# xubiker/deephisto

Hardware: AMD Instinct MI355X
Metric: 256x256 patches/sec WSI inference (predict_full_patched) (higher is better)
Workload: dtype bf16; 1 GPU; BASELINE configs[2]: predict_full_patched on one 50000x50000x3 closed-form synthetic WSI resident in HBM, 256x256 tiles stride 256, ResNet-18 (random init), bf16 MFMA, step = one whole slide (tile grid -> fused gather+forward -> all-gather -> ordered accumulate -> argmax); patch=256, stride=256, sampler_batch=64, micro_batch=4096, streams=1, downscale=16, n_tiles=38416, n_classes=5, parallelism=tile-range shard x1

## Files before the change

### deephisto_amd/_lib.py

```python
from __future__ import annotations

import ctypes as C
from pathlib import Path

import torch

LIB_PATH = Path(__file__).resolve().parent / "libdeephisto_hip.so"

DH_LAYOUT_NHWC, DH_LAYOUT_NCHW = 0, 1
DH_DTYPE_F32, DH_DTYPE_BF16 = 0, 1

_i32, _i64, _u32 = C.c_int32, C.c_int64, C.c_uint32
BUCKET_CB = C.CFUNCTYPE(None, C.c_int32, C.c_int64, C.c_int64, C.c_void_p)
_p = C.c_void_p

SIGNATURES = {
    "dh_abi_version": (C.c_int, []),
    "dh_last_error": (C.c_char_p, []),
    "dh_tile_grid_count": (C.c_int, [_i64, _i64, _i32, _i32, _i32, C.POINTER(_i64), C.POINTER(_i64)]),
    "dh_tile_grid": (C.c_int, [_i64, _i64, _i32, _i32, _i32, _p, _i64]),
    "dh_synth_slide": (C.c_int, [_p, _i64, _i64, _u32, _p]),
    "dh_tile_gather": (C.c_int, [_p, _i64, _i64, _p, _p, _i64, _i32, _i32, _i32, _p, _p]),
    "dh_tile_gather_aug": (C.c_int, [_p, _i64, _i64, _p, _i64, _i32, _i32, _i32, _i32, _i32, _p, _p]),
    "dh_tile_gather_raw": (C.c_int, [_p, _i64, _i64, _p, _i64, _i32, _p, _p]),
# ... 59 lines not shown
    "dh_train2_debug_act": (C.c_int, [_p, C.c_char_p, _i32, _p, _i64, _p]),
    "dh_debug_gemm1x1_bf16": (C.c_int, [_p, _p, _p, _p, _i64] + [_i32] * 8 + [_p]),
    "dh_debug_gemm1x1_fused_bf16": (C.c_int, [_p] * 7 + [_i64] + [_i32] * 8 + [_p]),
    "dh_debug_gemm1x1_bwdsums_bf16": (C.c_int, [_p] * 10 + [_i32, _p, _i64, _i32, _i32, _p]),
    "dh_debug_bn2_bf16": (C.c_int, [_p, _p, _p, _p, _i32, _p, _p, _p, _p, _i32, _p, _p, _p, _p, _i64, _i32, _p]),
    "dh_debug_stem_wgrad_bf16": (C.c_int, [_p, _p, _p, _i32, _i32, _p]),
    "dh_debug_bn2_pool_bf16": (C.c_int, [_p, _p, _p, _p, _p, _p, _p, _p, _p, _p, _p, _i32, _i32, _i32, _i32, _p]),
    "dh_debug_maxpool2_bf16": (C.c_int, [_p, _p, _p, _p, _i32, _i32, _i32, _i32, _p]),
    "dh_debug_upsample2_add_bf16": (C.c_int, [_p, _p] + [_i32] * 6 + [_p]),
    "dh_debug_avgpool_fc_dgrad2": (C.c_int, [_p, _p, _p] + [_i32] * 4 + [_p]),
    "dh_debug_wgrad_bf16": (C.c_int, [_p, _p, _p] + [_i32] * 8 + [_p]),
    "dh_debug_conv_bn_act": (C.c_int, [_p, _p, _p, _p, _p, _p] + [_i32] * 9 + [_p]),
    "dh_debug_stem_out": (C.c_int, [_p, _i64, _i32, _p, _p]),
    "dh_debug_stem_pool_bf16": (C.c_int, [_p, _p, _i64, _i64, _p, _i64, _i32, _p, _p]),
    "dh_debug_wgrad_f32": (C.c_int, [_p, _p, _p] + [_i32] * 8 + [_p]),
    "dh_debug_stem_wgrad_f32": (C.c_int, [_p, _p, _p, _i32, _i32, _p]),
    "dh_debug_dgrad_f32": (C.c_int, [_p, _p, _p, _p] + [_i32] * 7 + [_p]),
    "dh_debug_pack_f32": (C.c_int, [_p, _i32, _i32, _p, _p, _p, _p, _p]),
    "dh_debug_pack_bf16": (C.c_int, [_p, _i32, _i32, _p, _p, _p, _p, _p]),
    "dh_debug_bn_f32": (C.c_int, [_p, _p, _p, _p, _i32, _p, _p, _p, _p, _p, _p, _p, _i64, _i32, _p]),
    "dh_debug_maxpool_f32": (C.c_int, [_p, _p, _p, _p, _i32, _i32, _i32, _i32, _p]),
    "dh_debug_bn_pool_f32": (C.c_int, [_p, _p, _p, _p, _p, _p, _p, _p, _p, _i32, _i32, _i32, _i32, _p]),
    "dh_debug_stamps": (C.c_int, [_i32, _p]),
    "dh_debug_env_knobs": (C.c_int, [C.c_char_p, _i64]),
    "dh_debug_coverage_set_map": (C.c_int, [_p, _p, _p]),
    "dh_debug_resnet18_forward_tap": (C.c_int, [_p, _p, _i64, _i64, _p, _i64, _i32, C.c_char_p, _p, _i32, _p, _i64, _p, _p]),
    "dh_debug_resnet50_forward_tap": (C.c_int, [_p, _p, _i64, _i64, _p, _i64, _i32, C.c_char_p, _p, _i32, _p, _i64, _p, _p]),
    "dh_debug_resnet18_operands": (C.c_int, [_p, C.c_char_p, _p, _i64, _p, _p, _i64]),
    "dh_debug_resnet50_operands": (C.c_int, [_p, C.c_char_p, _p, _i64, _p, _p, _i64]),
}


class DeephistoHipError(RuntimeError):
    pass


_lib = None


def lib() -> C.CDLL:
    global _lib
    if _lib is None:
        if not LIB_PATH.exists():
            raise DeephistoHipError(
                f"{LIB_PATH} is missing: build it with `python -m deephisto_amd.build` "
                "(hipcc --offload-arch=gfx950). There is no CPU fallback for the HIP path.")
# ... 13 lines not shown
```

### deephisto_amd/csrc/resnet50_infer.inc

```

constexpr int R50_MAX_P = 256;
constexpr int64_t R50_MAX_TILES = ((int64_t)1 << 31) / ((int64_t)256 * (R50_MAX_P / 4) * (R50_MAX_P / 4) * 2);
static_assert(R50_MAX_TILES == DH_RESNET50_MAX_TILES, "include/deephisto_hip.h states the launch limit");

struct dh_resnet50 {
  struct Blk { int c1 = -1, c2 = -1, c3 = -1, ds = -1, stride = 1; };
  int n_classes = 0;
  std::map<std::string, std::vector<float>> params;
  std::vector<ConvLayer> convs;
  std::vector<Blk> blocks;
  float* ones = nullptr;
  float* fc_w = nullptr;
  float* fc_b = nullptr;
  bool finalized = false;
  void* ws = nullptr;
  size_t ws_bytes = 0;
  std::vector<int32_t> yx_host;
};

namespace {

void r50_topology(dh_resnet50* net) {
  net->convs.clear(); net->blocks.clear();
  auto add = [&](const std::string& n, const std::string& bn, int cin, int cout, int ks, int stride) {
// ... 61 lines not shown
  DH_LAUNCH_CHECK();
  return DH_OK;
}

int r50_forward_impl(dh_resnet50* net, const float* x, const uint8_t* slide, int64_t slide_h, int64_t slide_w, const int32_t* yx,
                     int B, int P, float* logits, hipStream_t st, Tap* tap = nullptr) {
  const int H2 = P / 4;
  auto al = [](size_t v) { return (v + 255) & ~(size_t)255; };
  const size_t px = (size_t)B * H2 * H2 * 2;
  const size_t big = al(256 * px), t1 = al(128 * px), t2 = al(64 * px);
  const size_t need = 2 * big + t1 + t2;
  if (need > net->ws_bytes) {
    if (net->ws) DH_HIP(hipFree(net->ws));
    net->ws = nullptr; net->ws_bytes = 0;
    DH_HIP(hipMalloc(&net->ws, need));
    net->ws_bytes = need;
  }
  char* base = static_cast<char*>(net->ws);
  bf16_t* X = reinterpret_cast<bf16_t*>(base);
  bf16_t* D = reinterpret_cast<bf16_t*>(base + big);
  bf16_t* T1 = reinterpret_cast<bf16_t*>(base + 2 * big);
  bf16_t* T2 = reinterpret_cast<bf16_t*>(base + 2 * big + t1);
  int rc;
  if ((rc = launch_stem_pool(net->convs[0], x, slide, slide_h, slide_w, yx, B, P, X, st))) return rc;
  for (const char* nm : {"conv1", "maxpool"})
    if ((rc = tap_after<__bf16>(tap, nm, X, 64, H2, H2, 32, st))) return rc;
  int H = H2;
  for (const dh_resnet50::Blk& b : net->blocks) {
    const ConvLayer &c1 = net->convs[b.c1], &c2 = net->convs[b.c2], &c3 = net->convs[b.c3];
    const int Ho = (H - 1) / b.stride + 1;
    if ((rc = r50_gemm(c1, X, nullptr, T1, B, H, H, true, st))) return rc;
    if ((rc = tap_after<__bf16>(tap, c1.name, T1, c1.cout, H, H, 32, st))) return rc;
    rc = b.stride == 1 ? launch_conv3x3<__bf16, 1>(c2, T1, nullptr, T2, B, H, H, true, st, Ho, Ho, nullptr, nullptr, true)
                       : launch_conv3x3<__bf16, 2>(c2, T1, nullptr, T2, B, H, H, true, st, Ho, Ho, nullptr, nullptr, true);
    if (rc) return rc;
    if ((rc = tap_after<__bf16>(tap, c2.name, T2, c2.cout, Ho, Ho, 32, st))) return rc;
    const bf16_t* idt = X;
    if (b.ds >= 0) {
      if ((rc = r50_gemm(net->convs[b.ds], X, nullptr, D, B, H, H, false, st))) return rc;
      if ((rc = tap_after<__bf16>(tap, net->convs[b.ds].name, D, c3.cout, Ho, Ho, 32, st))) return rc;
      idt = D;
    }
    if ((rc = r50_gemm(c3, T2, idt, X, B, Ho, Ho, true, st))) return rc;
    if ((rc = tap_after<__bf16>(tap, c3.name, X, c3.cout, Ho, Ho, 32, st))) return rc;
    H = Ho;
  }
  hipLaunchKernelGGL(r50_head_kernel, dim3(B), dim3(256), 0, st, X, H * H, net->fc_w, net->fc_b, net->n_classes, logits);
// ... 160 lines not shown
```

### deephisto_amd/csrc/resnet_kernels.hip

```cpp
#include <math.h>
#include <stdlib.h>
#include <string.h>

#include <algorithm>
#include <array>
#include <map>
#include <mutex>
#include <set>
#include <string>
#include <vector>

#include "dh_common.h"
#include "conv3_tables_host.h"

typedef float f32x16 __attribute__((ext_vector_type(16)));
typedef __bf16 bf16x8 __attribute__((ext_vector_type(8)));

namespace {

constexpr int CHUNK_BYTES = 64;
constexpr int PIX_PITCH = 80;
constexpr int FRAG_BYTES = 1024;
constexpr int SLAB_TAP = 4 * FRAG_BYTES;

// ... 997 lines not shown
int run_conv(const ConvLayer& L, const void* in, const void* res, void* out, int B, int Hi, int Wi,
             bool relu, hipStream_t st, int* Ho_out, int* Wo_out, bool blocked = false, bool out16 = false) {
  const int pad = L.ks / 2;
  const int Ho = (Hi + 2 * pad - L.ks) / L.stride + 1, Wo = (Wi + 2 * pad - L.ks) / L.stride + 1;
  *Ho_out = Ho; *Wo_out = Wo;
  DH_REQUIRE((int64_t)B * Hi * Wi * L.cin * (int64_t)sizeof(T) < ((int64_t)1 << 32),
             "conv %s: input larger than 4 GiB, reduce the batch", L.name.c_str());
  if (L.ks == 3 && L.stride == 1) return launch_conv3x3<T, 1>(L, in, res, out, B, Hi, Wi, relu, st, Ho, Wo, nullptr, nullptr, blocked, 0, 0, false, out16);
  DH_REQUIRE(!out16, "conv %s: only the stride-1 3x3 kernel writes 16-channel planes", L.name.c_str());
  if (L.ks == 3 && L.stride == 2) return launch_conv3x3<T, 2>(L, in, res, out, B, Hi, Wi, relu, st, Ho, Wo, nullptr, nullptr, blocked);
  DH_REQUIRE(!blocked, "conv %s: only the 3x3 kernels read the channel-blocked layout", L.name.c_str());
  ConvParams p;
  p.in = in; p.w = L.w_dev; p.scale = L.scale_dev; p.shift = L.shift_dev; p.res = res; p.out = out;
  p.B = B; p.Hi = Hi; p.Wi = Wi; p.Cin = L.cin; p.Cout = L.cout; p.Ho = Ho; p.Wo = Wo;
  if (p.Ho > 8 || p.Wo > 8) { p.TH = 16; p.TW = 16; p.IMGS = 1; }
  else { p.TH = 8; p.TW = 8; p.IMGS = 4; }
  p.tiles_y = (p.Ho + p.TH - 1) / p.TH; p.tiles_x = (p.Wo + p.TW - 1) / p.TW;
  p.relu = relu ? 1 : 0;
  if (L.ks == 1 && L.stride == 2) return launch_conv<T, 1, 2, false>(p, st);
  dh::set_error("conv %s: unsupported shape", L.name.c_str());
  return DH_EINVAL;
}

int launch_stem_pool(const ConvLayer& stem, const float* x, const uint8_t* slide, int64_t slide_h, int64_t slide_w,
                     const int32_t* yx, int B, int P, void* out, hipStream_t st) {
  const int H1 = (P + 6 - 7) / 2 + 1, H2 = (H1 + 2 - 3) / 2 + 1;
  StemPoolParams sp;
  DH_REQUIRE(!slide || slide_w < (1 << 24), "stem: slide rows of %lld pixels are not supported (< 2^24)", (long long)slide_w);
  sp.x_nchw = x; sp.slide = slide; sp.yx = yx; sp.row_bytes = slide_w * 3; sp.slide_bytes = slide_h * slide_w * 3;
  sp.w = stem.w_dev; sp.scale = stem.scale_dev; sp.shift = stem.shift_dev; sp.out = out;
  sp.B = B; sp.P = P; sp.Hc = H1; sp.Wc = H1; sp.Hp = H2; sp.Wp = H2;
  sp.tiles_y = (H2 + SP_PR - 1) / SP_PR; sp.tiles_x = (H2 + SP_PC - 1) / SP_PC;
  sp.nstrips = B * sp.tiles_x;
  const int grid = std::min(768, sp.nstrips);
  sp.iters = ((sp.nstrips + grid - 1) / grid) * sp.tiles_y;
  int arc;
  if ((arc = ensure_dyn_lds(reinterpret_cast<const void*>(&stem_pool_kernel<true, false>), SP_LDS)) ||
      (arc = ensure_dyn_lds(reinterpret_cast<const void*>(&stem_pool_kernel<true, true>), SP_LDS)) ||
      (arc = ensure_dyn_lds(reinterpret_cast<const void*>(&stem_pool_kernel<false, false>), SP_LDS))) return arc;
  sp.stamps = nullptr;
  if (g_stamps_on && slide) {
    if (!g_stamps_dev) {
      DH_HIP(hipMalloc((void**)&g_stamps_dev, 64 * sizeof(unsigned long long)));
      DH_HIP(hipMemset(g_stamps_dev, 0, 64 * sizeof(unsigned long long)));
    }
    sp.stamps = g_stamps_dev + 8 * 7;
  }
  if (slide && sp.stamps) hipLaunchKernelGGL((stem_pool_kernel<true, true>), dim3(grid), dim3(SP_T), SP_LDS, st, sp);
  else if (slide) hipLaunchKernelGGL((stem_pool_kernel<true, false>), dim3(grid), dim3(SP_T), SP_LDS, st, sp);
  else hipLaunchKernelGGL((stem_pool_kernel<false, false>), dim3(grid), dim3(SP_T), SP_LDS, st, sp);
  DH_LAUNCH_CHECK();
  return DH_OK;
}

struct Tap {
  std::string name;
  const int32_t* sel = nullptr;
  int k = 0;
  float* out = nullptr;
  int64_t out_elems = 0;
  bool hit = false;
};

template <typename T>
__global__ void tap_gather_kernel(const T* __restrict__ in, const int32_t* __restrict__ sel, int C, int cp, int64_t hw, int64_t total,
                                  float* __restrict__ out) {
  for (int64_t i = (int64_t)blockIdx.x * blockDim.x + threadIdx.x; i < total; i += (int64_t)gridDim.x * blockDim.x) {
    const int64_t px = i % hw;
    const int c = (int)((i / hw) % C);
    const int64_t b = sel[i / hw / C];
    out[i] = (float)in[((b * (C / cp) + c / cp) * hw + px) * cp + c % cp];
  }
}

// ... 28 lines not shown
  const int esz = (int)sizeof(T);
  const int H1 = (P + 6 - 7) / 2 + 1;
  const int H2 = (H1 + 2 - 3) / 2 + 1;
  const size_t stem_bytes = (size_t)B * H1 * H1 * 64 * esz;
  const size_t act_bytes = (size_t)B * H2 * H2 * 64 * esz;
  DH_REQUIRE(act_bytes < ((size_t)1 << 32),
             "resnet18 forward: %d tiles of %d x %d in %s make an activation larger than 4 GiB: use fewer tiles per launch", B, P, P,
             sizeof(T) == 2 ? "bf16" : "float32");
  auto al = [](size_t v) { return (v + 255) & ~(size_t)255; };
  const size_t need = al(stem_bytes) + 3 * al(act_bytes);
  if (need > net->ws_bytes) {
    if (net->ws) DH_HIP(hipFree(net->ws));
    net->ws = nullptr; net->ws_bytes = 0;
    DH_HIP(hipMalloc(&net->ws, need));
    net->ws_bytes = need;
  }
  char* base = static_cast<char*>(net->ws);
  void* S = base;
  void* bufA = base + al(stem_bytes);
  void* bufB = base + al(stem_bytes) + al(act_bytes);
  void* bufC = base + al(stem_bytes) + 2 * al(act_bytes);

  if constexpr (sizeof(T) == 2) {
    if (int rc = launch_stem_pool(net->convs[0], x, slide, slide_h, slide_w, yx, B, P, bufA, st)) return rc;
    for (const char* nm : {"conv1", "maxpool"})
      if (int rc = tap_after<T>(tap, nm, bufA, 64, H2, H2, 32, st)) return rc;
  } else {
  {
    StemParams sp;
    sp.x_nchw = x; sp.slide = slide; sp.yx = yx; sp.row_bytes = slide_w * 3;
    sp.w = net->convs[0].w_dev; sp.scale = net->convs[0].scale_dev; sp.shift = net->convs[0].shift_dev;
    sp.out = S; sp.B = B; sp.P = P; sp.Ho = H1; sp.Wo = H1; sp.relu = 1;
    sp.tiles_y = (H1 + STEM_TH - 1) / STEM_TH; sp.tiles_x = (H1 + STEM_TW - 1) / STEM_TW;
    const size_t wb = esz == 2 ? (size_t)7 * 2 * 2 * FRAG_BYTES : (size_t)7 * 11 * 2 * 256;
    const size_t lds = wb + (size_t)STEM_ROWS * STEM_ROWE * esz;
    const int grid = B * sp.tiles_y * sp.tiles_x;
    if (slide) {
      if (int arc = ensure_dyn_lds(reinterpret_cast<const void*>(&stem_kernel<T, true>), 96 * 1024)) return arc;
      hipLaunchKernelGGL((stem_kernel<T, true>), dim3(grid), dim3(256), lds, st, sp);
    } else {
      if (int arc = ensure_dyn_lds(reinterpret_cast<const void*>(&stem_kernel<T, false>), 96 * 1024)) return arc;
      hipLaunchKernelGGL((stem_kernel<T, false>), dim3(grid), dim3(256), lds, st, sp);
    }
    DH_LAUNCH_CHECK();
    if (int rc = tap_after<T>(tap, "conv1", S, 64, H1, H1, 64, st)) return rc;
  }
  {
// ... 241 lines not shown
    hipLaunchKernelGGL((to_f32_kernel<__bf16>), dim3(1024), dim3(256), 0, st, static_cast<const __bf16*>(net->ws), out_dev, elems);
  DH_LAUNCH_CHECK();
  return DH_OK;
}

namespace {
__global__ void blocked_to_nhwc_f32_kernel(const __bf16* in, float* out, int64_t n, int hw) {
  const int64_t total = n * hw * 64;
  for (int64_t i = blockIdx.x * (int64_t)blockDim.x + threadIdx.x; i < total; i += (int64_t)gridDim.x * blockDim.x) {
    const int c = (int)(i % 64);
    const int64_t px = (i / 64) % hw, b = i / 64 / hw;
    out[i] = (float)in[((b * 2 + c / 32) * hw + px) * 32 + c % 32];
  }
}
}

extern "C" int dh_debug_stem_pool_bf16(dh_resnet18* net, const uint8_t* slide_dev, int64_t slide_h, int64_t slide_w,
                                       const int32_t* yx_dev, int64_t n, int32_t P, float* out_dev, void* stream) {
  DH_REQUIRE(net && net->finalized && net->dtype == DH_DTYPE_BF16, "debug stem pool: needs a finalized bf16 network");
  DH_REQUIRE(slide_dev && yx_dev && out_dev && n > 0 && n <= (1 << 20) && P >= 32 && P <= 1024, "debug stem pool: bad arguments");
  hipStream_t st = dh::as_stream(stream);
  const int H1 = (P + 6 - 7) / 2 + 1, H2 = (H1 + 2 - 3) / 2 + 1;
  void* tmp = nullptr;
  DH_HIP(hipMalloc(&tmp, (size_t)n * H2 * H2 * 64 * 2));
  int rc = launch_stem_pool(net->convs[0], nullptr, slide_dev, slide_h, slide_w, yx_dev, (int)n, P, tmp, st);
  if (!rc) {
    hipLaunchKernelGGL(blocked_to_nhwc_f32_kernel, dim3(1024), dim3(256), 0, st, static_cast<const __bf16*>(tmp), out_dev, n, H2 * H2);
    if (hipGetLastError() != hipSuccess) rc = DH_EHIP;
    (void)hipStreamSynchronize(st);
  }
  (void)hipFree(tmp);
  return rc;
}

namespace {
template <typename Net>
bool tap_name_known(const Net* net, const char* name) {
  if (!strcmp(name, "maxpool")) return true;
  for (const auto& c : net->convs)
    if (c.name == name) return true;
  return false;
}

int read_operands(const ConvLayer& c, int esz, bool fused_stem, float* w_host, int64_t w_elems, float* scale_host, float* shift_host,
                  int64_t c_elems) {
  DH_REQUIRE(w_host && scale_host && shift_host, "operands: null argument");
  DH_REQUIRE(w_elems == (int64_t)c.cout * c.cin * c.ks * c.ks && c_elems == c.cout, "operands %s: buffers of %lld / %lld elements, "
             "expected %lld / %d", c.name.c_str(), (long long)w_elems, (long long)c_elems, (long long)c.cout * c.cin * c.ks * c.ks, c.cout);
// ... 57 lines not shown
    float t = 0.f;
    DH_HIP(hipEventElapsedTime(&t, g_prof.ev[i], g_prof.ev[i + 1]));
    ms += t;
  }
  if (total_ms) *total_ms = ms;
  if (total_flops) *total_flops = g_prof.flops;
  if (n_samples) *n_samples = (int64_t)(g_prof.used / 2);
  for (hipEvent_t e : g_prof.ev) (void)hipEventDestroy(e);
  g_prof.ev.clear(); g_prof.used = 0;
  return DH_OK;
}

extern "C" int dh_debug_stamps(int32_t enable, unsigned long long* out64_host) {
  g_stamps_on = enable != 0;
  if (out64_host) {
    if (!g_stamps_dev) { memset(out64_host, 0, 64 * sizeof(unsigned long long)); return DH_OK; }
    DH_HIP(hipDeviceSynchronize());
    DH_HIP(hipMemcpy(out64_host, g_stamps_dev, 64 * sizeof(unsigned long long), hipMemcpyDeviceToHost));
    DH_HIP(hipMemset(g_stamps_dev, 0, 64 * sizeof(unsigned long long)));
  }
  return DH_OK;
}

#include "gemm1x1_f32.inc"
#include "train.inc"
#include "train2_kernels.inc"
#include "wgrad_ring.inc"
#include "bn_fold.inc"
#include "gemm1x1.inc"
#include "train2.inc"
#include "gemm1x1_infer.inc"
#include "resnet50_infer.inc"
```

### deephisto_amd/csrc/stem_pool.inc

```
#ifndef SP_ABL
#define SP_ABL 0
#endif
constexpr int SP_W = 4;
constexpr int SP_T = SP_W * 64;
constexpr int SP_CR = 2 * SP_W, SP_CC = 32;
constexpr int SP_PR = SP_W, SP_PC = 15;
constexpr int SP_WR = 2 * SP_CR + 5;
constexpr int SP_WE = 224;
#ifndef SP_PF
#define SP_PF 3
#endif
constexpr int SP_KS = 11;
constexpr int SP_WBYTES = SP_KS * 2 * FRAG_BYTES;
constexpr int SP_WINB = ((SP_WR * SP_WE * 2 + 255) / 256) * 256;
constexpr int SP_XCH = 4096;
constexpr int SP_LDS = SP_WBYTES + SP_WINB + (SP_W + 1) * SP_XCH + 512;
constexpr int SP_DW = 52;
constexpr int SP_NLOAD = (SP_WR * SP_DW + SP_T - 1) / SP_T;
static_assert(3 * ((SP_LDS + 511) / 512 * 512) <= 160 * 1024, "three workgroups per CU");

inline void sp_kslot(int ks, int hh, int j, int* kh, int* s) {
  *kh = -1; *s = 0;
  if (ks < 9) {
    const int pz = ks / 3, u = ks % 3;
    if (u == 0) { *kh = 2 * pz; *s = 8 * hh + j; }
    else if (u == 1) { *kh = 2 * pz + hh; *s = hh ? j : 16 + j; }
    else { *kh = 2 * pz + 1; *s = 8 + 8 * hh + j; }
  } else if (ks == 9) { *kh = 6; *s = 8 * hh + j; }
  else if (hh == 0) { *kh = 6; *s = 16 + j; }
}

struct StemPoolParams {
  const float* x_nchw; const uint8_t* slide; const int32_t* yx; int64_t row_bytes, slide_bytes;
  const void* w; const float* scale; const float* shift; void* out;
  int B, P, Hc, Wc, Hp, Wp, tiles_y, tiles_x, nstrips, iters;
  unsigned long long* stamps;
};

typedef unsigned short sp_u16x2 __attribute__((ext_vector_type(2)));

template <bool SRC_U8, bool STAMP>
__global__ __launch_bounds__(SP_T, 3) void stem_pool_kernel(const StemPoolParams p) {
  extern __shared__ __attribute__((aligned(16))) char smem[];
  char* w_lds = smem;
  char* win_lds = smem + SP_WBYTES;
  char* xch_lds = win_lds + SP_WINB;
  float* ss_lds = reinterpret_cast<float*>(xch_lds + (SP_W + 1) * SP_XCH);
  const int tid = threadIdx.x, lane = tid & 63, tx = lane & 31, h = lane >> 5;
  const int wave = __builtin_amdgcn_readfirstlane(tid >> 6);
  for (int i = wave; i < SP_WBYTES / 1024; i += SP_W)
    lds_dma<16>(static_cast<const char*>(p.w) + i * 1024 + lane * 16, __builtin_amdgcn_readfirstlane(lds_addr_of(w_lds + i * 1024)));
  if (tid < 128) ss_lds[tid] = tid < 64 ? p.scale[tid] : p.shift[tid - 64];
  for (int i = tid * 16; i < SP_WINB; i += SP_T * 16) *reinterpret_cast<uint4*>(win_lds + i) = make_uint4(0, 0, 0, 0);

  struct Tile { int valid, b, py0, px0, ty0, tx0, first; };
  int cur_sid = (int)blockIdx.x, cur_ty = 0, cur_b = cur_sid / p.tiles_x, cur_px0 = (cur_sid % p.tiles_x) * SP_PC, cur_it = 0;
  auto next_tile = [&]() __attribute__((always_inline)) {
    Tile t;
    t.valid = cur_sid < p.nstrips && cur_it < p.iters;
    t.b = cur_b; t.py0 = cur_ty * SP_PR; t.px0 = cur_px0; t.first = cur_ty == 0;
    t.ty0 = 0; t.tx0 = 0;
    if constexpr (SRC_U8) {
      if (t.valid) { t.ty0 = p.yx[2 * t.b]; t.tx0 = p.yx[2 * t.b + 1]; }
    }
    ++cur_it;
    if (++cur_ty == p.tiles_y) {
      cur_ty = 0; cur_sid += (int)gridDim.x;
      cur_b = cur_sid / p.tiles_x; cur_px0 = (cur_sid % p.tiles_x) * SP_PC;
    }
    return t;
  };

  constexpr int SP_TAIL = SP_WR * SP_DW - (SP_NLOAD - 1) * SP_T;
  uint32_t wr[SP_NLOAD], wr2[SP_NLOAD];
  uint32_t woff[SP_NLOAD];
  int wrd[SP_NLOAD];
  uint32_t colm[SP_NLOAD];
#pragma unroll
  for (int k = 0; k < SP_NLOAD; ++k) {
    wr[k] = 0; wr2[k] = 0; colm[k] = 0;
    const int idx = tid + k * SP_T;
    const bool own = idx < SP_WR * SP_DW;
    const int r = own ? idx / SP_DW : 0, d = own ? idx % SP_DW : 0;
    woff[k] = (uint32_t)(r * (int)p.row_bytes + 4 * d);
    wrd[k] = r << 8 | d;
  }
  struct __attribute__((packed, aligned(1))) U32 { uint32_t v; };
  auto load_window = [&](const Tile& t, uint32_t (&wr)[SP_NLOAD]) __attribute__((always_inline)) {
    if constexpr (SRC_U8) {
      const int iy0 = 4 * t.py0 - 3, ix0 = 4 * t.px0 - 5;
      const int64_t worg = (int64_t)(t.ty0 + iy0) * p.row_bytes + (int64_t)(t.tx0 + ix0) * 3 - 1;
      const int64_t wend = worg + (int64_t)(SP_WR - 1) * p.row_bytes + 4 * SP_DW;
      if constexpr (SP_ABL & 2) return;
      if (worg >= 0 && wend <= p.slide_bytes) {
        const uint8_t* base = p.slide + worg;
#pragma unroll
        for (int k = 0; k < SP_NLOAD; ++k) wr[k] = reinterpret_cast<const U32*>(base + ((SP_ABL & 64) ? (woff[k] & 1023u) : woff[k]))->v;
      } else {
#pragma unroll
        for (int k = 0; k < SP_NLOAD; ++k) {
          const int64_t a = worg + woff[k];
          uint32_t v = 0;
          for (int i = 0; i < 4; ++i)
            if (a + i >= 0 && a + i < p.slide_bytes) v |= (uint32_t)p.slide[a + i] << (8 * i);
          wr[k] = v;
        }
      }
    }
  };
  auto store_window = [&](const Tile& t, uint32_t (&wr)[SP_NLOAD]) __attribute__((always_inline)) {
    uint16_t* win = reinterpret_cast<uint16_t*>(win_lds);
    const int iy0 = 4 * t.py0 - 3, ix0 = 4 * t.px0 - 5;
    if constexpr (SRC_U8) {
      if constexpr (SP_ABL & 4) {
#pragma unroll
        for (int k = 0; k < SP_NLOAD; ++k) if (wr[k] == 0x12345678u) win[k] = 1;
        return;
      }
      if (t.first) {
        const int q_lo = max(0, -ix0) * 3, q_hi = min(207, (p.P - ix0) * 3);
#pragma unroll
        for (int k = 0; k < SP_NLOAD; ++k) {
          const int q0 = 4 * (wrd[k] & 255) - 1;
          const int lo = min(max(q_lo - q0, 0), 4), hi = min(max(q_hi - q0, 0), 4);
          colm[k] = (lo < 4 ? 0xFFFFFFFFu << (8 * lo) : 0u) & (hi > 0 ? 0xFFFFFFFFu >> (32 - 8 * hi) : 0u);
        }
      }
      if (!(ix0 >= 0 && ix0 + 69 <= p.P)) {
#pragma unroll
        for (int k = 0; k < SP_NLOAD; ++k) wr[k] &= colm[k];
      }
      if (!(iy0 >= 0 && iy0 + SP_WR <= p.P)) {
        const int r_lo = max(0, -iy0), r_hi = min(SP_WR, p.P - iy0);
#pragma unroll
        for (int k = 0; k < SP_NLOAD; ++k) {
          const int r = wrd[k] >> 8;
          if (r < r_lo || r >= r_hi) wr[k] = 0u;
        }
      }
#pragma unroll
      for (int k = 0; k < SP_NLOAD; ++k) {
        if (k < SP_NLOAD - 1 || tid < SP_TAIL) {
          const float r255 = 1.0f / 255.0f;
          const uint32_t w = wr[k];
          typedef __bf16 bf16x4_t __attribute__((ext_vector_type(4)));
          const bf16x4_t w4 = {(__bf16)((float)(w & 0xFFu) * r255), (__bf16)((float)((w >> 8) & 0xFFu) * r255),
                               (__bf16)((float)((w >> 16) & 0xFFu) * r255), (__bf16)((float)(w >> 24) * r255)};
          *reinterpret_cast<bf16x4_t*>(win + (wrd[k] >> 8) * SP_WE + 4 * (wrd[k] & 255)) = w4;
        }
      }
    } else {
      for (int idx = tid; idx < SP_WR * 207; idx += SP_T) {
        const int r = idx / 207, q = idx % 207;
        const int iy = iy0 + r, ix = ix0 + q / 3, c = q % 3;
        float v = 0.f;
        if (iy >= 0 && iy < p.P && ix >= 0 && ix < p.P) v = p.x_nchw[(((int64_t)t.b * 3 + c) * p.P + iy) * p.P + ix];
        win[r * SP_WE + 1 + q] = (uint16_t)f32_to_bf16(v);
      }
    }
  };

  Tile cur = next_tile();
  Tile nxt = next_tile();
  Tile nn = next_tile();
#ifdef SP_STAGGER
  {
    const int ph = (int)(blockIdx.x / 256u) % 3;
    for (int i = 0; i < ph * SP_STAGGER; ++i) __builtin_amdgcn_s_sleep(32);
  }
#endif
  asm volatile("s_waitcnt vmcnt(0)" ::: "memory");
  __syncthreads();
  if (cur.valid) { load_window(cur, wr); store_window(cur, wr); }
  if (nxt.valid) load_window(nxt, wr);
  __syncthreads();

  unsigned long long tacc[6] = {0, 0, 0, 0, 0, 0};
  unsigned long long tprev = STAMP ? __builtin_readcyclecounter() : 0ull;
  auto stamp = [&](int slot) __attribute__((always_inline)) {
    if constexpr (STAMP) {
      __builtin_amdgcn_sched_barrier(0);
      const unsigned long long now = __builtin_readcyclecounter();
      __builtin_amdgcn_sched_barrier(0);
      tacc[slot] += now - tprev;
      tprev = now;
    }
  };
  typedef short sp_i16x2 __attribute__((ext_vector_type(2)));
  auto max16 = [](uint32_t a, uint32_t b) __attribute__((always_inline)) {
    return __builtin_bit_cast(uint32_t, __builtin_elementwise_max(__builtin_bit_cast(sp_i16x2, a), __builtin_bit_cast(sp_i16x2, b)));
  };
  auto hmax3 = [&](uint32_t v0) __attribute__((always_inline)) {
    const uint32_t v1 = (uint32_t)__builtin_amdgcn_update_dpp(0, (int)v0, 0x130, 0xF, 0xF, true);
    const uint32_t v2 = (uint32_t)__builtin_amdgcn_update_dpp(0, (int)v1, 0x130, 0xF, 0xF, true);
    return max16(max16(v0, v1), v2);
  };
  const int xlane = lane * 64, xsw = (lane >> 2) & 3;
  const bool even = !(tx & 1);
  const char* a_base = w_lds + lane * 16;
  const int b_base = ((4 * wave) * SP_WE + 6 * tx) * 2;
  int b_off[3];
  b_off[0] = 16 * h;
  b_off[1] = h ? SP_WE * 2 : 32;
  b_off[2] = h ? 16 : 32;
  struct SpStep { int row, shift, sel, ka, kb; };
  constexpr SpStep SCHED[14] = {
      {0, 0, 0, 0, -1}, {0, 0, 1, 1, -1}, {1, 16, 0, 2, -1},
      {2, 0, 0, 3, 0},  {2, 0, 1, 4, 1},  {3, 16, 0, 5, 2},
      {4, 0, 0, 6, 3},  {4, 0, 1, 7, 4},  {5, 16, 0, 8, 5},
      {6, 0, 0, 9, 6},  {6, 0, 1, 10, 7}, {7, 16, 0, -1, 8},
      {8, 0, 0, -1, 9}, {8, 0, 2, -1, 10}};
  auto read_a = [&](int ks, int mt) __attribute__((always_inline)) {
    return (SP_ABL & 32) ? make_uint4(lane, tid, lane, lane) : *reinterpret_cast<const uint4*>(a_base + (ks * 2 + mt) * FRAG_BYTES);
  };
  auto read_b = [&](int f) __attribute__((always_inline)) {
    const uint32_t* src = reinterpret_cast<const uint32_t*>(win_lds + b_base + b_off[SCHED[f].sel] + SCHED[f].row * SP_WE * 2 + SCHED[f].shift);
    return (SP_ABL & 32) ? make_uint4(tid, tid, lane, tid) : make_uint4(src[0], src[1], src[2], src[3]);
  };
// ... 13 lines not shown
      };
#pragma unroll
      for (int f = 0; f < SP_PF; ++f) fetch(f);
#pragma unroll
      for (int f = 0; f < 14; ++f) {
        if (f + SP_PF < 14) fetch(f + SP_PF);
#pragma unroll
        for (int nt = 0; nt < 2; ++nt) {
          const int ks = nt == 0 ? SCHED[f].ka : SCHED[f].kb;
          if (ks < 0) continue;
#pragma unroll
          for (int mt = 0; mt < 2; ++mt) {
            if constexpr (SP_ABL & 1) {
              if (ks == 0) acc[mt][nt] = zero16;
              asm volatile("" :: "v"(wa[ks][mt].x), "v"(wa[ks][mt].y), "v"(wa[ks][mt].z), "v"(wa[ks][mt].w), "v"(bq[f % (SP_PF + 1)].x), "v"(bq[f % (SP_PF + 1)].y), "v"(bq[f % (SP_PF + 1)].z), "v"(bq[f % (SP_PF + 1)].w));
            } else {
              acc[mt][nt] = __builtin_amdgcn_mfma_f32_32x32x16_bf16(__builtin_bit_cast(bf16x8, wa[ks][mt]), __builtin_bit_cast(bf16x8, bq[f % (SP_PF + 1)]),
                                                                    ks == 0 ? zero16 : acc[mt][nt], 0, 0, 0);
            }
          }
        }
      }
      stamp(1);
      const int r0 = 2 * cur.py0, c0 = 2 * cur.px0 - 1;
      const bool interior = r0 + SP_CR <= p.Hc && c0 >= 0 && c0 + SP_CC <= p.Wc;
      char* slot = xch_lds + (wave < SP_W - 1 ? wave : SP_W - 1 + (it & 1)) * SP_XCH + xlane;
      auto bn_pack = [&](auto inside) __attribute__((always_inline)) {
        constexpr bool INSIDE = decltype(inside)::value;
        uint32_t okm[2] = {~0u, ~0u};
        if constexpr (!INSIDE) {
          const bool col_ok = (c0 + tx) >= 0 && (c0 + tx) < p.Wc;
          okm[0] = col_ok && (r0 + 2 * wave) < p.Hc ? ~0u : 0u;
          okm[1] = col_ok && (r0 + 2 * wave + 1) < p.Hc ? ~0u : 0u;
        }
        typedef float f32x2_t __attribute__((ext_vector_type(2)));
        typedef __bf16 bf16x2_t __attribute__((ext_vector_type(2)));
#pragma unroll
        for (int mt = 0; mt < 2; ++mt)
#pragma unroll
          for (int pr = 0; pr < 2; ++pr) {
            uint32_t rb[2][2];
#pragma unroll
            for (int gg = 0; gg < 2; ++gg) {
              const int g = 2 * pr + gg;
              const float4 sc = *reinterpret_cast<const float4*>(ss_lds + (mt * 4 + g) * 8 + 4 * h);
              const float4 sh = *reinterpret_cast<const float4*>(ss_lds + 64 + (mt * 4 + g) * 8 + 4 * h);
              uint32_t row[2][2];
// ... 6 lines not shown
                if constexpr (!INSIDE) { row[nt][0] &= okm[nt]; row[nt][1] &= okm[nt]; }
              }
              rb[gg][0] = row[1][0]; rb[gg][1] = row[1][1];
              vm[mt][g][0] = max16(row[0][0], row[1][0]);
              vm[mt][g][1] = max16(row[0][1], row[1][1]);
            }
            *reinterpret_cast<uint4*>(slot + (((mt * 2 + pr) ^ xsw) << 4)) = make_uint4(rb[0][0], rb[0][1], rb[1][0], rb[1][1]);
          }
      };
      if (interior) bn_pack(std::true_type{});
      else bn_pack(std::false_type{});
      stamp(2);
    }
    asm volatile("s_waitcnt lgkmcnt(0)" ::: "memory");
    __builtin_amdgcn_s_barrier();
    asm volatile("" ::: "memory");
    stamp(5);
    if (nxt.valid) store_window(nxt, wnow);
    stamp(4);
    if (cur.valid) {
      const char* prev = xch_lds + (wave > 0 ? wave - 1 : SP_W - 1 + ((it + 1) & 1)) * SP_XCH + xlane;
      const bool have_prev = wave > 0 || !cur.first;
      const int py = cur.py0 + wave, px = cur.px0 + (tx >> 1);
      const bool st_ok = even && (tx >> 1) < SP_PC && py < p.Hp && px < p.Wp;
      const int plane = p.Hp * p.Wp * 32;
      __bf16* out = static_cast<__bf16*>(p.out) + (int64_t)cur.b * 2 * plane + (py * p.Wp + px) * 32;
      uint4 pvq[4];
#pragma unroll
      for (int q = 0; q < 4; ++q) pvq[q] = make_uint4(0u, 0u, 0u, 0u);
      if (have_prev) {
#pragma unroll
        for (int q = 0; q < 4; ++q) pvq[q] = *reinterpret_cast<const uint4*>(prev + ((q ^ xsw) << 4));
      }
#pragma unroll
      for (int mt = 0; mt < 2; ++mt)
#pragma unroll
        for (int pr = 0; pr < 2; ++pr) {
          const uint4 pv = pvq[mt * 2 + pr];
          uint32_t v[4] = {max16(vm[mt][2 * pr][0], pv.x), max16(vm[mt][2 * pr][1], pv.y),
                           max16(vm[mt][2 * pr + 1][0], pv.z), max16(vm[mt][2 * pr + 1][1], pv.w)};
          if constexpr (!(SP_ABL & 8)) {
#pragma unroll
            for (int i = 0; i < 4; ++i) v[i] = max16(hmax3(v[i]), 0u);
          }
          uint32_t a0 = v[0], a1 = v[1], b0 = v[2], b1 = v[3];
          { const auto r = __builtin_amdgcn_permlane32_swap(a0, b0, false, false); a0 = r[0]; b0 = r[1]; }
          { const auto r = __builtin_amdgcn_permlane32_swap(a1, b1, false, false); a1 = r[0]; b1 = r[1]; }
          if constexpr (SP_ABL & 16) asm volatile("" :: "v"(a0), "v"(a1), "v"(b0), "v"(b1));
          else if (st_ok) *reinterpret_cast<uint4*>(out + mt * plane + (2 * pr + h) * 8) = make_uint4(a0, a1, b0, b1);
        }
      stamp(3);
    }
    asm volatile("s_waitcnt lgkmcnt(0)" ::: "memory");
    __builtin_amdgcn_s_barrier();
    asm volatile("" ::: "memory");
    stamp(5);
    cur = nxt;
    nxt = nn;
    nn = n3;
  };
  for (int it = 0; it < p.iters; it += 2) {
    step(it, wr, wr2);
    step(it + 1, wr2, wr);
  }
  if constexpr (STAMP) {
    if (tid == 0 && p.stamps) {
      for (int i = 0; i < 6; ++i) atomicAdd(p.stamps + i, tacc[i]);
      atomicAdd(p.stamps + 6, 1ull);
    }
  }
}
```

### include/deephisto_hip_debug.h

```cpp
#ifndef DEEPHISTO_HIP_DEBUG_H
#define DEEPHISTO_HIP_DEBUG_H

#include "deephisto_hip.h"

#ifdef __cplusplus
extern "C" {
#endif

int dh_train2_debug_act(dh_train2* net, const char* conv_name, int32_t what, float* out_dev, int64_t n_elem, void* stream);

int dh_debug_pack_bf16(const float* w_dev, int32_t cout, int32_t cin, uint16_t* wf_tile, uint16_t* wd_tile, uint16_t* wf_elem,
                       uint16_t* wd_elem, void* stream);
int dh_debug_gemm1x1_bf16(const uint16_t* a_dev, const uint16_t* w_dev, const uint16_t* res_dev, uint16_t* out_dev, int64_t M,
                          int32_t N, int32_t K, int32_t stride, int32_t Ho, int32_t Wo, int32_t Hi, int32_t Wi, int32_t repeat,
                          void* stream);
int dh_debug_gemm1x1_fused_bf16(const uint16_t* a_dev, const uint16_t* w_dev, const uint16_t* res_dev, const uint16_t* mask_dev,
                                uint16_t* out_dev, float* mean_dev, float* invstd_dev, int64_t M, int32_t N, int32_t K, int32_t stride,
                                int32_t Ho, int32_t Wo, int32_t Hi, int32_t Wi, int32_t repeat, void* stream);
int dh_debug_gemm1x1_bwdsums_bf16(const uint16_t* a_dev, const uint16_t* w_dev, const uint16_t* res_dev, const uint16_t* mask_dev,
                                  uint16_t* out_dev, const uint16_t* z_dev, const float* mean_dev, const float* invstd_dev,
                                  const float* scale_dev, const float* shift_dev, int32_t relu_mode, float* sums_dev, int64_t M, int32_t N,
                                  int32_t K, void* stream);
int dh_debug_bn2_bf16(const uint16_t* z_dev, const uint16_t* res_dev, const float* gamma_dev, const float* beta_dev, int32_t relu,
                      uint16_t* y_dev, float* mean_dev, float* invstd_dev, const uint16_t* dy_dev, int32_t relu_mode, uint16_t* dz_dev,
// ... 13 lines not shown

int dh_debug_conv_bn_act(const void* in_dev, const float* w_host, const float* scale_host,
                         const float* shift_host, const void* res_dev, void* out_dev, int32_t B,
                         int32_t H, int32_t W, int32_t cin, int32_t cout, int32_t ks, int32_t stride,
                         int32_t relu, int32_t dtype, void* stream);
int dh_debug_stem_out(dh_resnet18* net, int64_t n, int32_t patch, float* out_dev, void* stream);
int dh_debug_stem_pool_bf16(dh_resnet18* net, const uint8_t* slide_dev, int64_t slide_h, int64_t slide_w, const int32_t* yx_dev,
                            int64_t n, int32_t patch, float* out_dev, void* stream);
int dh_debug_wgrad_f32(const float* dz_dev, const float* x_dev, float* dw_dev, int32_t B, int32_t Hi, int32_t Wi,
                       int32_t cin, int32_t cout, int32_t ks, int32_t stride, int32_t mode, void* stream);
int dh_debug_stem_wgrad_f32(const float* dz_dev, const float* x_nchw_dev, float* dw_dev, int32_t B, int32_t P, void* stream);
int dh_debug_dgrad_f32(const float* dz_dev, const float* w_dev, const float* res_dev, float* dx_dev, int32_t B, int32_t Hi,
                       int32_t Wi, int32_t cin, int32_t cout, int32_t ks, int32_t stride, void* stream);
int dh_debug_pack_f32(const float* w_dev, int32_t cout, int32_t cin, float* wf_tile, float* wd_tile, float* wf_elem, float* wd_elem,
                      void* stream);
int dh_debug_bn_f32(const float* z_dev, const float* gamma_dev, const float* beta_dev, const float* res_dev, int32_t relu,
                    float* y_dev, const float* dy_dev, float* dz_dev, float* g_dev, float* dgamma_dev, float* dbeta_dev,
                    float* stats_out_dev, int64_t rows, int32_t C, void* stream);
int dh_debug_maxpool_f32(const float* x_dev, float* y_dev, const float* dy_dev, float* dx_dev, int32_t B, int32_t Hi, int32_t Wi,
                         int32_t C, void* stream);
int dh_debug_bn_pool_f32(const float* z_dev, const float* gamma_dev, const float* beta_dev, float* pooled_dev, uint8_t* idx_dev,
                         const float* dpool_dev, float* dz_dev, float* dgamma_dev, float* dbeta_dev, int32_t B, int32_t Hi, int32_t Wi,
                         int32_t C, void* stream);
int dh_debug_stamps(int32_t enable, unsigned long long* out64_host);
int dh_debug_env_knobs(char* buf_host, int64_t cap);

int dh_debug_resnet18_forward_tap(dh_resnet18* net, const uint8_t* slide, int64_t h, int64_t w, const int32_t* yx_dev, int64_t n, int32_t P,
                                  const char* conv_name, const int32_t* sel_dev, int32_t k, float* out_dev, int64_t out_elems,
                                  float* logits_dev, void* stream);
int dh_debug_resnet50_forward_tap(dh_resnet50* net, const uint8_t* slide, int64_t h, int64_t w, const int32_t* yx_dev, int64_t n, int32_t P,
                                  const char* conv_name, const int32_t* sel_dev, int32_t k, float* out_dev, int64_t out_elems,
                                  float* logits_dev, void* stream);
int dh_debug_resnet18_operands(dh_resnet18* net, const char* conv_name, float* w_host, int64_t w_elems, float* scale_host,
                               float* shift_host, int64_t c_elems);
int dh_debug_resnet50_operands(dh_resnet50* net, const char* conv_name, float* w_host, int64_t w_elems, float* scale_host,
                               float* shift_host, int64_t c_elems);

int dh_debug_coverage_set_map(dh_coverage* cov, const int32_t* map_host, void* stream);

#ifdef __cplusplus
}
#endif
#endif
```

Baseline: 220,500 patches/s.

## Use 16-column stem strips with a seam fixup pass instead of overlapping 15-column strips

The fused stem conv+BN+ReLU+maxpool kernel previously tiled pooled output into strips of 15 columns, which recomputes halo columns so each strip can pool alone. The strip width is now chosen at runtime and is 16 when that gives fewer strips, as it does for 256 patches (4 strips instead of 5 per row). Each strip then pools only its own columns. The left neighbour's contribution to the column at each strip boundary is saved in a seam scratch buffer, and a small follow-up kernel max-merges it into the output. This removes redundant stem compute and window loads, but adds a second kernel launch, extra seam scratch traffic and more index logic.

```diff
diff --git a/deephisto_amd/_lib.py b/deephisto_amd/_lib.py
--- a/deephisto_amd/_lib.py
+++ b/deephisto_amd/_lib.py
@@ -105,6 +105,7 @@
     "dh_debug_maxpool_f32": (C.c_int, [_p, _p, _p, _p, _i32, _i32, _i32, _i32, _p]),
     "dh_debug_bn_pool_f32": (C.c_int, [_p, _p, _p, _p, _p, _p, _p, _p, _p, _i32, _i32, _i32, _i32, _p]),
     "dh_debug_stamps": (C.c_int, [_i32, _p]),
+    "dh_debug_stem_strip_width": (C.c_int, [_i32]),
     "dh_debug_env_knobs": (C.c_int, [C.c_char_p, _i64]),
     "dh_debug_coverage_set_map": (C.c_int, [_p, _p, _p]),
     "dh_debug_resnet18_forward_tap": (C.c_int, [_p, _p, _i64, _i64, _p, _i64, _i32, C.c_char_p, _p, _i32, _p, _i64, _p, _p]),
diff --git a/deephisto_amd/csrc/resnet50_infer.inc b/deephisto_amd/csrc/resnet50_infer.inc
--- a/deephisto_amd/csrc/resnet50_infer.inc
+++ b/deephisto_amd/csrc/resnet50_infer.inc
@@ -107,7 +107,8 @@
   bf16_t* T1 = reinterpret_cast<bf16_t*>(base + 2 * big);
   bf16_t* T2 = reinterpret_cast<bf16_t*>(base + 2 * big + t1);
   int rc;
-  if ((rc = launch_stem_pool(net->convs[0], x, slide, slide_h, slide_w, yx, B, P, X, st))) return rc;
+  DH_REQUIRE(stem_seam_bytes(B, P) <= t1, "resnet50 forward: seam scratch larger than the bottleneck buffer");
+  if ((rc = launch_stem_pool(net->convs[0], x, slide, slide_h, slide_w, yx, B, P, X, T1, st))) return rc;
   for (const char* nm : {"conv1", "maxpool"})
     if ((rc = tap_after<__bf16>(tap, nm, X, 64, H2, H2, 32, st))) return rc;
   int H = H2;
diff --git a/deephisto_amd/csrc/resnet_kernels.hip b/deephisto_amd/csrc/resnet_kernels.hip
--- a/deephisto_amd/csrc/resnet_kernels.hip
+++ b/deephisto_amd/csrc/resnet_kernels.hip
@@ -1043,22 +1043,48 @@
   return DH_EINVAL;
 }
 
+int g_stem_pc_force = 0;
+
+int stem_pool_pc(int P) {
+  const int H1 = (P + 6 - 7) / 2 + 1, H2 = (H1 + 2 - 3) / 2 + 1;
+  if (g_stem_pc_force) return g_stem_pc_force;
+  return (H2 + 15) / 16 < (H2 + 14) / 15 ? 16 : 15;
+}
+
+size_t stem_seam_bytes(int B, int P) {
+  const int H1 = (P + 6 - 7) / 2 + 1, H2 = (H1 + 2 - 3) / 2 + 1;
+  return stem_pool_pc(P) == 16 ? (size_t)B * ((H2 + 15) / 16 - 1) * H2 * 64 * 2 : 0;
+}
+
+template <int PC>
+int launch_stem_pool_pc(const StemPoolParams& sp, int grid, hipStream_t st) {
+  int arc;
+  if ((arc = ensure_dyn_lds(reinterpret_cast<const void*>(&stem_pool_kernel<true, false, PC>), SP_LDS)) ||
+      (arc = ensure_dyn_lds(reinterpret_cast<const void*>(&stem_pool_kernel<true, true, PC>), SP_LDS)) ||
+      (arc = ensure_dyn_lds(reinterpret_cast<const void*>(&stem_pool_kernel<false, false, PC>), SP_LDS))) return arc;
+  if (sp.slide && sp.stamps) hipLaunchKernelGGL((stem_pool_kernel<true, true, PC>), dim3(grid), dim3(SP_T), SP_LDS, st, sp);
+  else if (sp.slide) hipLaunchKernelGGL((stem_pool_kernel<true, false, PC>), dim3(grid), dim3(SP_T), SP_LDS, st, sp);
+  else hipLaunchKernelGGL((stem_pool_kernel<false, false, PC>), dim3(grid), dim3(SP_T), SP_LDS, st, sp);
+  DH_LAUNCH_CHECK();
+  return DH_OK;
+}
+
 int launch_stem_pool(const ConvLayer& stem, const float* x, const uint8_t* slide, int64_t slide_h, int64_t slide_w,
-                     const int32_t* yx, int B, int P, void* out, hipStream_t st) {
+                     const int32_t* yx, int B, int P, void* out, void* seam, hipStream_t st) {
   const int H1 = (P + 6 - 7) / 2 + 1, H2 = (H1 + 2 - 3) / 2 + 1;
+  const int pc = stem_pool_pc(P);
   StemPoolParams sp;
   DH_REQUIRE(!slide || slide_w < (1 << 24), "stem: slide rows of %lld pixels are not supported (< 2^24)", (long long)slide_w);
   sp.x_nchw = x; sp.slide = slide; sp.yx = yx; sp.row_bytes = slide_w * 3; sp.slide_bytes = slide_h * slide_w * 3;
   sp.w = stem.w_dev; sp.scale = stem.scale_dev; sp.shift = stem.shift_dev; sp.out = out;
   sp.B = B; sp.P = P; sp.Hc = H1; sp.Wc = H1; sp.Hp = H2; sp.Wp = H2;
-  sp.tiles_y = (H2 + SP_PR - 1) / SP_PR; sp.tiles_x = (H2 + SP_PC - 1) / SP_PC;
+  sp.tiles_y = (H2 + SP_PR - 1) / SP_PR; sp.tiles_x = (H2 + pc - 1) / pc;
+  sp.seam = seam;
+  const int nseam = pc == 16 ? sp.tiles_x - 1 : 0;
+  DH_REQUIRE(!nseam || seam, "stem: %d strips of 16 pooled columns need a seam scratch", sp.tiles_x);
   sp.nstrips = B * sp.tiles_x;
   const int grid = std::min(768, sp.nstrips);
   sp.iters = ((sp.nstrips + grid - 1) / grid) * sp.tiles_y;
-  int arc;
-  if ((arc = ensure_dyn_lds(reinterpret_cast<const void*>(&stem_pool_kernel<true, false>), SP_LDS)) ||
-      (arc = ensure_dyn_lds(reinterpret_cast<const void*>(&stem_pool_kernel<true, true>), SP_LDS)) ||
-      (arc = ensure_dyn_lds(reinterpret_cast<const void*>(&stem_pool_kernel<false, false>), SP_LDS))) return arc;
   sp.stamps = nullptr;
   if (g_stamps_on && slide) {
     if (!g_stamps_dev) {
@@ -1067,10 +1093,13 @@
     }
     sp.stamps = g_stamps_dev + 8 * 7;
   }
-  if (slide && sp.stamps) hipLaunchKernelGGL((stem_pool_kernel<true, true>), dim3(grid), dim3(SP_T), SP_LDS, st, sp);
-  else if (slide) hipLaunchKernelGGL((stem_pool_kernel<true, false>), dim3(grid), dim3(SP_T), SP_LDS, st, sp);
-  else hipLaunchKernelGGL((stem_pool_kernel<false, false>), dim3(grid), dim3(SP_T), SP_LDS, st, sp);
-  DH_LAUNCH_CHECK();
+  if (int rc = pc == 16 ? launch_stem_pool_pc<16>(sp, grid, st) : launch_stem_pool_pc<15>(sp, grid, st)) return rc;
+  if (nseam) {
+    const int64_t total = (int64_t)B * nseam * H2 * 8;
+    hipLaunchKernelGGL(stem_seam_kernel, dim3((unsigned)((total + 255) / 256)), dim3(256), 0, st, static_cast<const void*>(seam),
+                       static_cast<__bf16*>(out), total, nseam, H2, H2);
+    DH_LAUNCH_CHECK();
+  }
   return DH_OK;
 }
 
@@ -1145,7 +1174,8 @@
   void* bufC = base + al(stem_bytes) + 2 * al(act_bytes);
 
   if constexpr (sizeof(T) == 2) {
-    if (int rc = launch_stem_pool(net->convs[0], x, slide, slide_h, slide_w, yx, B, P, bufA, st)) return rc;
+    DH_REQUIRE(stem_seam_bytes(B, P) <= al(stem_bytes), "resnet18 forward: seam scratch larger than the stem slot");
+    if (int rc = launch_stem_pool(net->convs[0], x, slide, slide_h, slide_w, yx, B, P, bufA, S, st)) return rc;
     for (const char* nm : {"conv1", "maxpool"})
       if (int rc = tap_after<T>(tap, nm, bufA, 64, H2, H2, 32, st)) return rc;
   } else {
@@ -1433,8 +1463,10 @@
   hipStream_t st = dh::as_stream(stream);
   const int H1 = (P + 6 - 7) / 2 + 1, H2 = (H1 + 2 - 3) / 2 + 1;
   void* tmp = nullptr;
-  DH_HIP(hipMalloc(&tmp, (size_t)n * H2 * H2 * 64 * 2));
-  int rc = launch_stem_pool(net->convs[0], nullptr, slide_dev, slide_h, slide_w, yx_dev, (int)n, P, tmp, st);
+  auto al = [](size_t v) { return (v + 255) & ~(size_t)255; };
+  const size_t out_bytes = al((size_t)n * H2 * H2 * 64 * 2);
+  DH_HIP(hipMalloc(&tmp, out_bytes + stem_seam_bytes((int)n, P) + 256));
+  int rc = launch_stem_pool(net->convs[0], nullptr, slide_dev, slide_h, slide_w, yx_dev, (int)n, P, tmp, static_cast<char*>(tmp) + out_bytes, st);
   if (!rc) {
     hipLaunchKernelGGL(blocked_to_nhwc_f32_kernel, dim3(1024), dim3(256), 0, st, static_cast<const __bf16*>(tmp), out_dev, n, H2 * H2);
     if (hipGetLastError() != hipSuccess) rc = DH_EHIP;
@@ -1538,6 +1570,12 @@
   return DH_OK;
 }
 
+extern "C" int dh_debug_stem_strip_width(int32_t pc) {
+  DH_REQUIRE(pc == 0 || pc == 15 || pc == 16, "debug stem strip width: %d is not 0, 15 or 16", pc);
+  g_stem_pc_force = pc;
+  return DH_OK;
+}
+
 #include "gemm1x1_f32.inc"
 #include "train.inc"
 #include "train2_kernels.inc"
diff --git a/deephisto_amd/csrc/stem_pool.inc b/deephisto_amd/csrc/stem_pool.inc
--- a/deephisto_amd/csrc/stem_pool.inc
+++ b/deephisto_amd/csrc/stem_pool.inc
@@ -4,7 +4,7 @@
 constexpr int SP_W = 4;
 constexpr int SP_T = SP_W * 64;
 constexpr int SP_CR = 2 * SP_W, SP_CC = 32;
-constexpr int SP_PR = SP_W, SP_PC = 15;
+constexpr int SP_PR = SP_W;
 constexpr int SP_WR = 2 * SP_CR + 5;
 constexpr int SP_WE = 224;
 #ifndef SP_PF
@@ -33,14 +33,17 @@
 struct StemPoolParams {
   const float* x_nchw; const uint8_t* slide; const int32_t* yx; int64_t row_bytes, slide_bytes;
   const void* w; const float* scale; const float* shift; void* out;
+  void* seam;
   int B, P, Hc, Wc, Hp, Wp, tiles_y, tiles_x, nstrips, iters;
   unsigned long long* stamps;
 };
 
 typedef unsigned short sp_u16x2 __attribute__((ext_vector_type(2)));
 
-template <bool SRC_U8, bool STAMP>
+template <bool SRC_U8, bool STAMP, int PC>
 __global__ __launch_bounds__(SP_T, 3) void stem_pool_kernel(const StemPoolParams p) {
+  static_assert(PC == 15 || PC == 16, "strips of 15 or 16 pooled columns");
+  constexpr int CX = 16 - PC;
   extern __shared__ __attribute__((aligned(16))) char smem[];
   char* w_lds = smem;
   char* win_lds = smem + SP_WBYTES;
@@ -54,7 +57,7 @@
   for (int i = tid * 16; i < SP_WINB; i += SP_T * 16) *reinterpret_cast<uint4*>(win_lds + i) = make_uint4(0, 0, 0, 0);
 
   struct Tile { int valid, b, py0, px0, ty0, tx0, first; };
-  int cur_sid = (int)blockIdx.x, cur_ty = 0, cur_b = cur_sid / p.tiles_x, cur_px0 = (cur_sid % p.tiles_x) * SP_PC, cur_it = 0;
+  int cur_sid = (int)blockIdx.x, cur_ty = 0, cur_b = cur_sid / p.tiles_x, cur_px0 = (cur_sid % p.tiles_x) * PC, cur_it = 0;
   auto next_tile = [&]() __attribute__((always_inline)) {
     Tile t;
     t.valid = cur_sid < p.nstrips && cur_it < p.iters;
@@ -66,7 +69,7 @@
     ++cur_it;
     if (++cur_ty == p.tiles_y) {
       cur_ty = 0; cur_sid += (int)gridDim.x;
-      cur_b = cur_sid / p.tiles_x; cur_px0 = (cur_sid % p.tiles_x) * SP_PC;
+      cur_b = cur_sid / p.tiles_x; cur_px0 = (cur_sid % p.tiles_x) * PC;
     }
     return t;
   };
@@ -74,7 +77,7 @@
   constexpr int SP_TAIL = SP_WR * SP_DW - (SP_NLOAD - 1) * SP_T;
   uint32_t wr[SP_NLOAD], wr2[SP_NLOAD];
   uint32_t woff[SP_NLOAD];
-  int wrd[SP_NLOAD];
+  uint32_t wdst[SP_NLOAD];
   uint32_t colm[SP_NLOAD];
 #pragma unroll
   for (int k = 0; k < SP_NLOAD; ++k) {
@@ -83,12 +86,17 @@
     const bool own = idx < SP_WR * SP_DW;
     const int r = own ? idx / SP_DW : 0, d = own ? idx % SP_DW : 0;
     woff[k] = (uint32_t)(r * (int)p.row_bytes + 4 * d);
-    wrd[k] = r << 8 | d;
+    wdst[k] = (uint32_t)((r * SP_WE + 4 * d) * 2);
   }
+  auto piece_rd = [&](int k, int* r, int* d) __attribute__((always_inline)) {
+    uint32_t w = wdst[k];
+    asm volatile("" : "+v"(w));
+    *r = (int)(w / (uint32_t)(SP_WE * 2)); *d = (int)(w % (uint32_t)(SP_WE * 2)) >> 3;
+  };
   struct __attribute__((packed, aligned(1))) U32 { uint32_t v; };
   auto load_window = [&](const Tile& t, uint32_t (&wr)[SP_NLOAD]) __attribute__((always_inline)) {
     if constexpr (SRC_U8) {
-      const int iy0 = 4 * t.py0 - 3, ix0 = 4 * t.px0 - 5;
+      const int iy0 = 4 * t.py0 - 3, ix0 = 4 * t.px0 - 2 * CX - 3;
       const int64_t worg = (int64_t)(t.ty0 + iy0) * p.row_bytes + (int64_t)(t.tx0 + ix0) * 3 - 1;
       const int64_t wend = worg + (int64_t)(SP_WR - 1) * p.row_bytes + 4 * SP_DW;
       if constexpr (SP_ABL & 2) return;
@@ -110,7 +118,7 @@
   };
   auto store_window = [&](const Tile& t, uint32_t (&wr)[SP_NLOAD]) __attribute__((always_inline)) {
     uint16_t* win = reinterpret_cast<uint16_t*>(win_lds);
-    const int iy0 = 4 * t.py0 - 3, ix0 = 4 * t.px0 - 5;
+    const int iy0 = 4 * t.py0 - 3, ix0 = 4 * t.px0 - 2 * CX - 3;
     if constexpr (SRC_U8) {
       if constexpr (SP_ABL & 4) {
 #pragma unroll
@@ -121,7 +129,9 @@
         const int q_lo = max(0, -ix0) * 3, q_hi = min(207, (p.P - ix0) * 3);
 #pragma unroll
         for (int k = 0; k < SP_NLOAD; ++k) {
-          const int q0 = 4 * (wrd[k] & 255) - 1;
+          int r, d;
+          piece_rd(k, &r, &d);
+          const int q0 = 4 * d - 1;
           const int lo = min(max(q_lo - q0, 0), 4), hi = min(max(q_hi - q0, 0), 4);
           colm[k] = (lo < 4 ? 0xFFFFFFFFu << (8 * lo) : 0u) & (hi > 0 ? 0xFFFFFFFFu >> (32 - 8 * hi) : 0u);
         }
@@ -134,7 +144,8 @@
         const int r_lo = max(0, -iy0), r_hi = min(SP_WR, p.P - iy0);
 #pragma unroll
         for (int k = 0; k < SP_NLOAD; ++k) {
-          const int r = wrd[k] >> 8;
+          int r, d;
+          piece_rd(k, &r, &d);
           if (r < r_lo || r >= r_hi) wr[k] = 0u;
         }
       }
@@ -146,7 +157,7 @@
           typedef __bf16 bf16x4_t __attribute__((ext_vector_type(4)));
           const bf16x4_t w4 = {(__bf16)((float)(w & 0xFFu) * r255), (__bf16)((float)((w >> 8) & 0xFFu) * r255),
                                (__bf16)((float)((w >> 16) & 0xFFu) * r255), (__bf16)((float)(w >> 24) * r255)};
-          *reinterpret_cast<bf16x4_t*>(win + (wrd[k] >> 8) * SP_WE + 4 * (wrd[k] & 255)) = w4;
+          *reinterpret_cast<bf16x4_t*>(win_lds + wdst[k]) = w4;
         }
       }
     } else {
@@ -192,8 +203,13 @@
   };
   auto hmax3 = [&](uint32_t v0) __attribute__((always_inline)) {
     const uint32_t v1 = (uint32_t)__builtin_amdgcn_update_dpp(0, (int)v0, 0x130, 0xF, 0xF, true);
-    const uint32_t v2 = (uint32_t)__builtin_amdgcn_update_dpp(0, (int)v1, 0x130, 0xF, 0xF, true);
-    return max16(max16(v0, v1), v2);
+    if constexpr (PC == 16) {
+      const uint32_t vl = (uint32_t)__builtin_amdgcn_update_dpp(0, (int)v0, 0x138, 0xF, 0xF, true);
+      return max16(max16(v0, v1), tx == 0 ? 0u : vl);
+    } else {
+      const uint32_t v2 = (uint32_t)__builtin_amdgcn_update_dpp(0, (int)v1, 0x130, 0xF, 0xF, true);
+      return max16(max16(max16(v0, v1), v2), 0u);
+    }
   };
   const int xlane = lane * 64, xsw = (lane >> 2) & 3;
   const bool even = !(tx & 1);
@@ -253,7 +269,7 @@
         }
       }
       stamp(1);
-      const int r0 = 2 * cur.py0, c0 = 2 * cur.px0 - 1;
+      const int r0 = 2 * cur.py0, c0 = 2 * cur.px0 - CX;
       const bool interior = r0 + SP_CR <= p.Hc && c0 >= 0 && c0 + SP_CC <= p.Wc;
       char* slot = xch_lds + (wave < SP_W - 1 ? wave : SP_W - 1 + (it & 1)) * SP_XCH + xlane;
       auto bn_pack = [&](auto inside) __attribute__((always_inline)) {
@@ -306,9 +322,13 @@
       const char* prev = xch_lds + (wave > 0 ? wave - 1 : SP_W - 1 + ((it + 1) & 1)) * SP_XCH + xlane;
       const bool have_prev = wave > 0 || !cur.first;
       const int py = cur.py0 + wave, px = cur.px0 + (tx >> 1);
-      const bool st_ok = even && (tx >> 1) < SP_PC && py < p.Hp && px < p.Wp;
+      const bool st_ok = even && (tx >> 1) < PC && py < p.Hp && px < p.Wp;
       const int plane = p.Hp * p.Wp * 32;
       __bf16* out = static_cast<__bf16*>(p.out) + (int64_t)cur.b * 2 * plane + (py * p.Wp + px) * 32;
+      const bool seam_ok = PC == 16 && tx == 31 && py < p.Hp && cur.px0 + PC < p.Wp;
+      __bf16* seam = nullptr;
+      if constexpr (PC == 16)
+        seam = static_cast<__bf16*>(p.seam) + (((int64_t)cur.b * (p.tiles_x - 1) + cur.px0 / PC) * p.Hp + py) * 64;
       uint4 pvq[4];
 #pragma unroll
       for (int q = 0; q < 4; ++q) pvq[q] = make_uint4(0u, 0u, 0u, 0u);
@@ -323,9 +343,16 @@
           const uint4 pv = pvq[mt * 2 + pr];
           uint32_t v[4] = {max16(vm[mt][2 * pr][0], pv.x), max16(vm[mt][2 * pr][1], pv.y),
                            max16(vm[mt][2 * pr + 1][0], pv.z), max16(vm[mt][2 * pr + 1][1], pv.w)};
+          if constexpr (PC == 16) {
+#pragma unroll
+            for (int i = 0; i < 4; ++i) v[i] = max16(v[i], 0u);
+            if constexpr (!(SP_ABL & 16)) {
+              if (seam_ok) *reinterpret_cast<uint4*>(seam + h * 32 + mt * 16 + pr * 8) = make_uint4(v[0], v[1], v[2], v[3]);
+            }
+          }
           if constexpr (!(SP_ABL & 8)) {
 #pragma unroll
-            for (int i = 0; i < 4; ++i) v[i] = max16(hmax3(v[i]), 0u);
+            for (int i = 0; i < 4; ++i) v[i] = hmax3(v[i]);
           }
           uint32_t a0 = v[0], a1 = v[1], b0 = v[2], b1 = v[3];
           { const auto r = __builtin_amdgcn_permlane32_swap(a0, b0, false, false); a0 = r[0]; b0 = r[1]; }
@@ -354,3 +381,18 @@
     }
   }
 }
+
+__global__ __launch_bounds__(256) void stem_seam_kernel(const void* __restrict__ seam, __bf16* __restrict__ out, int64_t total,
+                                                        int nseam, int Hp, int Wp) {
+  typedef short sp_i16x8 __attribute__((ext_vector_type(8)));
+  const int64_t i = (int64_t)blockIdx.x * blockDim.x + threadIdx.x;
+  if (i >= total) return;
+  const int c8 = (int)(i & 7);
+  const int64_t px = i >> 3;
+  const int py = (int)(px % Hp), s = (int)((px / Hp) % nseam);
+  const int64_t b = px / Hp / nseam;
+  uint4* o = reinterpret_cast<uint4*>(out + (((b * 2 + (c8 >> 2)) * Hp + py) * Wp + 16 * (s + 1)) * 32 + (c8 & 3) * 8);
+  const uint2* row = reinterpret_cast<const uint2*>(seam) + px * 16 + c8;
+  const uint2 lo = row[0], hi = row[8];
+  *o = __builtin_bit_cast(uint4, __builtin_elementwise_max(__builtin_bit_cast(sp_i16x8, *o), __builtin_bit_cast(sp_i16x8, make_uint4(lo.x, lo.y, hi.x, hi.y))));
+}
diff --git a/include/deephisto_hip_debug.h b/include/deephisto_hip_debug.h
--- a/include/deephisto_hip_debug.h
+++ b/include/deephisto_hip_debug.h
@@ -59,6 +59,7 @@
 int dh_debug_bn_pool_f32(const float* z_dev, const float* gamma_dev, const float* beta_dev, float* pooled_dev, uint8_t* idx_dev,
                          const float* dpool_dev, float* dz_dev, float* dgamma_dev, float* dbeta_dev, int32_t B, int32_t Hi, int32_t Wi,
                          int32_t C, void* stream);
+int dh_debug_stem_strip_width(int32_t pooled_columns);
 int dh_debug_stamps(int32_t enable, unsigned long long* out64_host);
 int dh_debug_env_knobs(char* buf_host, int64_t cap);
 
```

Measured after the change: 223,400 patches/s, median of 6. +1.3%, better.
